# MoonLab-YH/AOD_MEH_HUA

Hardware: AMD Instinct MI355X
Metric: images/sec train+HUA-score, RetinaNet-R50 VOC 512^2 (higher is better)
Workload: dtype bf16x3

## Files before the change

### aod_meh_hua_amd/_C.py

```python
import ctypes as C
import os

import torch

_HERE = os.path.dirname(os.path.abspath(__file__))
LIB_PATH = os.environ.get('AOD_HIP_LIB') or os.path.join(_HERE, 'lib', 'libaodhip.so')


class AodHipError(RuntimeError):
    pass


if not os.path.exists(LIB_PATH):
    raise ImportError(f'{LIB_PATH} is missing: run `python -m aod_meh_hua_amd.build` (hipcc, gfx950). '
                      'There is no CPU fallback for the MEH/HUA hot path.')
lib = C.CDLL(LIB_PATH)


class ConvSeg(C.Structure):
    _fields_ = [('B', C.c_int32), ('H', C.c_int32), ('W', C.c_int32), ('OH', C.c_int32), ('OW', C.c_int32),
                ('src_row0', C.c_int64), ('dst_row0', C.c_int64)]


class ConvDesc(C.Structure):
# ... 42 lines not shown
    'aod_conv2d_plan': (C.c_int, [C.POINTER(ConvDesc), I32, C.c_uint, C.POINTER(ConvPlan)]),
    'aod_conv2d_grouped': (C.c_int, [C.POINTER(ConvDesc), I32, P, P, P, P, P, P, P]),
    'aod_conv2d_ws_map': (C.c_int, [C.POINTER(ConvDesc), P, P, P, P, P, P, P, P, P, P, P, SZ, P, P, P]),
    'aod_conv2d_grouped_map': (C.c_int, [C.POINTER(ConvDesc), I32, P, P, P, P, P, P, P, P, P]),
    'aod_fwd_row_maps': (C.c_int, [C.POINTER(ConvDesc), P, I32, I32, P, P]),
    'aod_conv2d_grouped_fwd_map': (C.c_int, [C.POINTER(ConvDesc), I32, P, P, P, P, P, P]),
    'aod_conv2d_grouped_deal': (C.c_int, [I32, I32, I32, P, P]),
    'aod_conv2d_grouped_map_order': (C.c_int, [C.POINTER(ConvDesc), I32, P, P, P, P, P, P, P, P, P, P]),
    'aod_conv2d_grouped_fwd_map_order': (C.c_int, [C.POINTER(ConvDesc), I32, P, P, P, P, P, P, P]),
    'aod_conv2d_tile_order': (C.c_int, [I32, I32, I32, P, P, P]),
    'aod_halo_conv3x3_applies': (C.c_int, [C.POINTER(ConvDesc)]),
    'aod_halo_conv3x3': (C.c_int, [C.POINTER(ConvDesc), P, P, P, P, P, P, P]),
    'aod_conv2d_wgrad': (C.c_int, [C.POINTER(ConvDesc), P, P, P, P, P]),
    'aod_conv2d_wgrad_splits': (C.c_int, [C.POINTER(ConvDesc)]),
    'aod_conv2d_wgrad_slabs': (C.c_int, [C.POINTER(ConvDesc), P, P, P, I32, I64, P, P]),
    'aod_conv2d_wgrad_slabs_map': (C.c_int, [C.POINTER(ConvDesc), P, P, P, I32, I64, P, P, P]),
    'aod_conv2d_wgrad_group_plan': (C.c_int, [P, I32, P]),
    'aod_conv2d_wgrad_grouped': (C.c_int, [P, I32, P, P, P, P, P, P, P]),
    'aod_conv2d_wgrad_plan': (C.c_int, [P, I32, P, P, P]),
    'aod_conv2d_wgrad_plan_ex': (C.c_int, [P, I32, C.c_uint, C.POINTER(WgradPlan)]),
    'aod_conv2d_wgrad_grouped_map': (C.c_int, [P, I32, P, P, P, P, P, P, P, P]),
    'aod_unpack_wgrad_slabs_grouped': (C.c_int, [I32, P, P, P, P, P, P, P, P, P, P, P, P, P, P, P, P, P]),
    'aod_unpack_wgrad_slabs': (C.c_int, [P, I32, I64, P, I32, I32, I32, I32, I32, I32, P, P, P, P, P, P, P]),
    'aod_conv_row_table_bytes': (SZ, [C.POINTER(ConvDesc)]),
    'aod_conv_row_table': (C.c_int, [C.POINTER(ConvDesc), P, P]),
    'aod_pack_weight_fwd': (C.c_int, [P, P, I32, I32, I32, I32, I32, P]),
    'aod_param_prep': (C.c_int, [P, I32, I32, P]),
    'aod_param_prep_item_bytes': (C.c_int, []),
    'aod_pack_weight_dgrad': (C.c_int, [P, P, I32, I32, I32, I32, I32, P, P]),
    'aod_unpack_wgrad': (C.c_int, [P, P, I32, I32, I32, I32, I32, I32, I32, P, P, P, P, P, P, P]),
    'aod_nchw_f32_to_nhwc_bf16': (C.c_int, [P, P, I32, I32, I32, I32, I32, P]),
    'aod_nchw_f32_to_s2d_bf16': (C.c_int, [P, P, I32, I32, I32, I32, P]),
    'aod_stem_pool_fwd': (C.c_int, [P, P, P, P, P, I32, I32, I32, P]),
    'aod_set_deterministic': (C.c_int, [I32]),
    'aod_get_deterministic': (C.c_int, []),
    'aod_stem_pool_x3_fwd': (C.c_int, [P, P, P, P, P, I32, I32, I32, I32, P]),
    'aod_maxpool3x3s2': (C.c_int, [P, P, I32, I32, I32, I32, P]),
    'aod_upsample2x_add': (C.c_int, [P, P, I32, I32, I32, I32, I32, I32, P]),
    'aod_upsample2x_add_bwd': (C.c_int, [P, P, I32, I32, I32, I32, I32, I32, P]),
    'aod_upsample2x_add_to': (C.c_int, [P, P, P, I32, I32, I32, I32, I32, I32, P]),
    'aod_upsample2x_add_bwd_set': (C.c_int, [P, P, I32, I32, I32, I32, I32, I32, P]),
    'aod_act_bwd': (C.c_int, [P, P, P, P, P, P, P, P, P, P, I64, I32, I32, I32, P]),
    'aod_add_relu': (C.c_int, [P, P, P, I64, P]),
    'aod_pad_cast_colsum': (C.c_int, [P, P, P, P, I64, I32, I32, I32, P]),
    'aod_assign_ws_bytes': (SZ, [I32, I32]),
    'aod_max_iou_assign': (C.c_int, [P, P, I64, I32, P, P, P, I32, F32, F32, F32, I32, I32, P, P, P, P, P, P, P, P, P, I32, P, P]),
# ... 104 lines not shown
```

### aod_meh_hua_amd/csrc/conv.hip

```cpp
#include "common.h"
#include "pointwise.h"
#include "conv_x3p.h"
#include "conv_params.h"

#ifdef AOD_TILE_TIMING
__device__ unsigned long long* g_tile_stamps = nullptr;
extern "C" int aod_dbg_set_tile_stamps(void* buf) { return (int)hipMemcpyToSymbol(HIP_SYMBOL(g_tile_stamps), &buf, sizeof(buf)); }
#define TSTAMP(k) do { if (g_tile_stamps && threadIdx.x == 0) g_tile_stamps[(size_t)blockIdx.x * 16 + (k)] = wall_clock64(); } while (0)
#else
#define TSTAMP(k) do {} while (0)
#endif

__device__ __forceinline__ unsigned udiv_small(unsigned n, unsigned d) {
  unsigned q = (unsigned)((float)n * __builtin_amdgcn_rcpf((float)d));
  const int r = (int)(n - q * d);
  q = r < 0 ? q - 1 : ((unsigned)r >= d ? q + 1 : q);
  return q;
}

__host__ __device__ __forceinline__ void conv_grouped_deal(int bid, int nwg, int ngroups, int mapped, int& tile, int& group) {
  if (!mapped) {
    const int wg = xcd_swizzle(bid, nwg * ngroups);
    tile = wg % nwg; group = wg / nwg;
    return;
// ... 1613 lines not shown
    const float v = dw[si];
    if (clear) dw[si] = 0.f;
    if (w) dot += w[gi] * v;
    g[gi] = accumulate ? g[gi] + v * sc : v * sc;
  }
  if (wdot) {
    dot = wave_sum(dot);
    if ((threadIdx.x & 63) == 0) red[threadIdx.x >> 6] = dot;
    __syncthreads();
    if (threadIdx.x == 0) {
      const float d = red[0] + red[1] + red[2] + red[3];
      wdot[oo] = bn_s1 ? bn_invstd[oo] * (d - bn_mean[oo] * bn_s1[oo]) : d;
    }
  }
}
constexpr int UNP_CH = 1024;
constexpr int UNP_T = 1024;
struct UnpackArgs {
  const float* dw; float* g; const float* scale; const float* w; float* wdot; const float* bn_s1; const float* bn_mean; const float* bn_invstd;
  long long slab_stride;
  int nslabs, O, I, RS, Ipad, accumulate;
  int x3;
};
__device__ __forceinline__ void unpack_row(const UnpackArgs& a, int oo, float* tile, float* red) {
  const float* __restrict__ dw = a.dw;
  float* __restrict__ g = a.g;
  const float* __restrict__ w = a.w;
  const int nslabs = a.nslabs, I = a.I, RS = a.RS, Ipad = a.Ipad, accumulate = a.accumulate;
  const long long slab_stride = a.slab_stride;
  const float sc = a.scale ? a.scale[oo] : 1.f;
  float dot = 0.f;
  const int CH = RS <= 9 ? UNP_CH : (UNP_CH * 9) / RS;
  for (int c0 = 0; c0 < I; c0 += CH) {
    const int nc = min(CH, I - c0);
    for (int i = threadIdx.x; i < nc * RS; i += UNP_T) {
      const int rs = i / nc, c = i - rs * nc;
      float v0 = 0.f, v1 = 0.f, v2 = 0.f, v3 = 0.f;
      {
      const float* src = dw + ((long long)oo * RS + rs) * Ipad + c0 + c;
      int sl = 0;
      for (; sl + 4 <= nslabs; sl += 4) {
        const float a0 = src[(long long)sl * slab_stride], a1 = src[(long long)(sl + 1) * slab_stride];
        const float a2 = src[(long long)(sl + 2) * slab_stride], a3 = src[(long long)(sl + 3) * slab_stride];
        v0 += a0; v1 += a1; v2 += a2; v3 += a3;
      }
      for (; sl < nslabs; ++sl) v0 += src[(long long)sl * slab_stride];
      }
      tile[c * RS + rs] = (v0 + v1) + (v2 + v3);
    }
    __syncthreads();
    const long long g0 = ((long long)oo * I + c0) * RS;
    for (int i = threadIdx.x; i < nc * RS; i += UNP_T) {
      const float v = tile[i];
      if (w) dot += w[g0 + i] * v;
      g[g0 + i] = accumulate ? g[g0 + i] + v * sc : v * sc;
    }
    __syncthreads();
  }
  if (a.wdot) {
    dot = wave_sum(dot);
    if ((threadIdx.x & 63) == 0) red[threadIdx.x >> 6] = dot;
    __syncthreads();
    if (threadIdx.x == 0) {
      float d = 0.f;
      for (int k = 0; k < UNP_T / 64; ++k) d += red[k];
      a.wdot[oo] = a.bn_s1 ? a.bn_invstd[oo] * (d - a.bn_mean[oo] * a.bn_s1[oo]) : d;
    }
  }
}
__global__ __launch_bounds__(UNP_T) void unpack_wgrad_slabs_kernel(const UnpackArgs a) {
  __shared__ float tile[UNP_CH * 9 + 1];
  __shared__ float red[UNP_T / 64];
  unpack_row(a, blockIdx.x, tile, red);
}
struct UnpackGroups { UnpackArgs g[WG_MAXG]; int blk0[WG_MAXG + 1]; };
__global__ __launch_bounds__(UNP_T) void unpack_wgrad_slabs_grouped_kernel(const UnpackGroups gp) {
  __shared__ float tile[UNP_CH * 9 + 1];
  __shared__ float red[UNP_T / 64];
  const int b = blockIdx.x;
  if (b < gp.blk0[1]) unpack_row(gp.g[0], b, tile, red);
  else if (b < gp.blk0[2]) unpack_row(gp.g[1], b - gp.blk0[1], tile, red);
  else if (b < gp.blk0[3]) unpack_row(gp.g[2], b - gp.blk0[2], tile, red);
  else unpack_row(gp.g[3], b - gp.blk0[3], tile, red);
}
struct PrepItem {
  const float* w; const float* gamma; const float* beta; const float* mean; const float* var;
  bf16_t* wf; bf16_t* wd; float* scale; float* shift; float* invstd;
  int O, I, RS, Ipad, Opad, blk0;
  float eps; int flags;
  long long pad2_[2];
};
constexpr int PREP_T = 32, PREP_RS = 9;
__global__ __launch_bounds__(256) void param_prep_kernel(const PrepItem* __restrict__ items, int nitems) {
  __shared__ float tile[PREP_RS][PREP_T][PREP_T + 1];
  int lo = 0, hi = nitems - 1;
  while (lo < hi) {
    const int mid = (lo + hi + 1) >> 1;
    if (items[mid].blk0 <= (int)blockIdx.x) lo = mid; else hi = mid - 1;
  }
  const PrepItem it = items[lo];
  const int lb = blockIdx.x - it.blk0;
  const int t = threadIdx.x;
  if (it.RS > PREP_RS) {
    const long long nf = (long long)it.O * it.RS * it.Ipad, nd = it.wd ? (long long)it.I * it.RS * it.Opad : 0;
    for (int u = 0; u < 8; ++u) {
      const long long i = (long long)lb * 2048 + u * 256 + t;
// ... 155 lines not shown
                                              const float* const* bn_mean, const float* const* bn_invstd, aod_stream_t stream) {
  AOD_CHECK_ARG(n >= 1 && n <= WG_MAXG && dw_slabs && nslabs && slab_stride && g && O && I && R && S && Ipad && accumulate && scale &&
                w_oihw && wdot && bn_s1 && bn_mean && bn_invstd, "unpack_wgrad_slabs_grouped: 1..4 members, no null arrays");
  UnpackGroups gp;
  memset(&gp, 0, sizeof(gp));
  int blk = 0;
  for (int i = 0; i < n; ++i) {
    AOD_CHECK_ARG(dw_slabs[i] && g[i] && nslabs[i] >= 1 && slab_stride[i] > 0 && O[i] >= 1, "unpack_wgrad_slabs_grouped: null / empty member");
    AOD_CHECK_ARG(R[i] * S[i] <= 16, "unpack_wgrad_slabs_grouped: at most 16 taps");
    AOD_CHECK_ARG(!wdot[i] || w_oihw[i], "unpack_wgrad_slabs_grouped: wdot needs the weights");
    AOD_CHECK_ARG(!bn_s1[i] || (wdot[i] && bn_mean[i] && bn_invstd[i]), "unpack_wgrad_slabs_grouped: BN mode needs wdot, mean and invstd");
    UnpackArgs& a = gp.g[i];
    a.dw = dw_slabs[i]; a.g = g[i]; a.scale = scale[i]; a.w = w_oihw[i]; a.wdot = wdot[i]; a.bn_s1 = bn_s1[i]; a.bn_mean = bn_mean[i];
    a.bn_invstd = bn_invstd[i];
    a.slab_stride = slab_stride[i]; a.nslabs = nslabs[i]; a.O = O[i]; a.I = I[i]; a.RS = R[i] * S[i]; a.Ipad = Ipad[i]; a.accumulate = accumulate[i] & 1; a.x3 = (accumulate[i] >> 1) & 1;
    gp.blk0[i] = blk;
    blk += O[i];
  }
  for (int i = n; i <= WG_MAXG; ++i) gp.blk0[i] = i == n ? blk : 0x7fffffff;
  hipLaunchKernelGGL(unpack_wgrad_slabs_grouped_kernel, dim3(blk), dim3(UNP_T), 0, (hipStream_t)stream, gp);
  AOD_LAUNCH_CHECK();
  return 0;
}
extern "C" int aod_unpack_wgrad(float* dw, float* g, int O, int I, int R, int S, int Ipad, int accumulate, int clear_src, const float* scale,
                                const float* w_oihw, float* wdot, const float* bn_s1, const float* bn_mean, const float* bn_invstd,
                                aod_stream_t stream) {
  AOD_CHECK_ARG(dw && g, "unpack_wgrad: null");
  AOD_CHECK_ARG(!wdot || w_oihw, "unpack_wgrad: wdot needs the weights");
  AOD_CHECK_ARG(!bn_s1 || (wdot && bn_mean && bn_invstd), "unpack_wgrad: BN mode needs wdot, mean and invstd");
  if (O == 0) return 0;
  hipLaunchKernelGGL(unpack_wgrad_kernel, dim3(O), dim3(256), 0, (hipStream_t)stream, dw, g, scale, w_oihw, wdot, bn_s1, bn_mean, bn_invstd, O, I,
                     R * S, Ipad, accumulate, clear_src);
  AOD_LAUNCH_CHECK();
  return 0;
}
```

### aod_meh_hua_amd/functional.py

```python
import torch
from torch.autograd import Function

from . import hipops as ho
from .hipops import Seg


def as_rows(x):
    B, C, H, W = x.shape
    xr = x.permute(0, 2, 3, 1)
    if not xr.is_contiguous():
        xr = xr.contiguous()
    return xr.view(B * H * W, C)


def as_nchw(rows, B, H, W):
    return rows.view(B, H, W, rows.shape[1]).permute(0, 3, 1, 2)


def multi_rows(tensors):
    rows = [as_rows(t) for t in tensors]
    if len(rows) == 1:
        t = tensors[0]
        return rows[0], [Seg(t.shape[0], t.shape[2], t.shape[3], 0)]
    rb = rows[0].shape[1] * rows[0].element_size()
# ... 345 lines not shown
MAP_LOG = None
FWD_MAP_LOG = None


def _map_of(dz):
    e = _ROW_MAPS.get(dz.data_ptr())
    return e[0] if e is not None and e[1].shape == dz.shape and e[1].dtype == dz.dtype and ho.sparse_bwd() else None


def _keep_map(dx, rmap):
    if rmap is not None:
        if MAP_LOG is not None:
            MAP_LOG.append((tuple(dx.shape), rmap))
        _WgradQueue.begin_pass()
        _ROW_MAPS[dx.data_ptr()] = (rmap, dx)


class _WgradQueue:
    jobs, seen, task, deferred = [], set(), -1, []
    sparse_jobs = []
    enabled = _os.environ.get('AOD_WGRAD_GROUP', '1') != '0'

    @classmethod
    def flush(cls):
        for name in ('jobs', 'sparse_jobs'):
            jobs = getattr(cls, name)
            setattr(cls, name, [])
            if jobs:
                ho.wgrad_unpack_group(jobs)

    @classmethod
    def _verify(cls):
        deferred, cls.deferred = cls.deferred, []
        for _, pref, t in deferred:
            p = pref()
            if p is None or p.grad is None:
                continue
            g = p.grad
            if g.data_ptr() != t.data_ptr() and g.shape == t.shape:
                g.copy_(t)

    @classmethod
    def _end_of_pass(cls):
        cls.task = -1
        cls.seen.clear()
        _S1_OF.clear()
        _ROW_MAPS.clear()
        cls.flush()
        cls._verify()

    @classmethod
    def begin_pass(cls):
        tid = torch._C._current_graph_task_id()
        if tid != cls.task:
            cls.flush()
            cls.deferred = []
            cls.task = tid
            cls.seen.clear()
            _S1_OF.clear()
            _ROW_MAPS.clear()
            if tid >= 0:
                torch.autograd.Variable._execution_engine.queue_callback(cls._end_of_pass)

    @classmethod
    def submit(cls, job, wid, defer):
        cls.begin_pass()
        if wid in cls.seen or not (defer and cls.enabled) or ho.DETERMINISTIC:
            cls.flush()
            job.run_alone()
            cls.deferred = [e for e in cls.deferred if e[0] != wid]
            cls.seen.add(wid)
            return False
        cls.seen.add(wid)
        name = 'sparse_jobs' if job.zmap is not None else 'jobs'
        q = getattr(cls, name)
        if q and ho.wgrad_group_splits(q + [job]) is None:
            setattr(cls, name, [])
            ho.wgrad_unpack_group(q)
            q = getattr(cls, name)
        q.append(job)
        if len(q) == 4:
            setattr(cls, name, [])
            ho.wgrad_unpack_group(q)
        return True


def _wgrad(x_rows, x_segs, dz, dsegs, R, S, stride, pad, dil, alg, w, O, I, dst, scale=None, bn=None, gamma=None, zmap=None):
    dev = dz.device
    gw = dst if dst is not None else torch.empty(O, I, R, S, dtype=torch.float32, device=dev)
    wdot = torch.empty(O, dtype=torch.float32, device=dev) if bn is not None else None
    job = ho.WgradJob(x_rows, x_segs, dz, dsegs, R, S, stride, pad, dil, alg, O, I, gw.detach(), scale=scale,
                      w=w.detach() if bn is not None else None, wdot=wdot.detach() if wdot is not None else None,
                      bn=tuple(t.detach() for t in bn) if bn is not None else None, zmap=zmap)
    hooked = lambda p: p is not None and bool(p._backward_hooks or getattr(p, '_post_accumulate_grad_hooks', None))
    defer = (R * S <= 9 and w.grad is None and (gamma is None or gamma.grad is None) and not torch.is_grad_enabled()
             and not torch.is_anomaly_enabled() and not hooked(w) and not hooked(gamma))
    if _WgradQueue.submit(job, id(w), defer):
        _WgradQueue.deferred.append((id(w), _weakref.ref(w), job.gw))
        if job.wdot is not None and gamma is not None:
            _WgradQueue.deferred.append((id(w), _weakref.ref(gamma), job.wdot))
    return gw, wdot


class ConvFn(Function):

    @staticmethod
# ... 893 lines not shown
```

### aod_meh_hua_amd/graphs.py

```python
import torch

from . import functional as AF
from . import hipops as ho
from .datasets import DeviceImageBatch

torch.autograd.graph.set_warn_on_accumulate_grad_stream_mismatch(False)
from .models.dense_heads.L_anchor_head import PackedGT


def _pin_caches():
    from . import scoring
    return (dict(ho._ROW_TABLES), dict(ho._DW), dict(ho._SLABS), list(AF.PREP.items.values()), AF.PREP.table, dict(scoring._META))


def _low_memory(dev, frac=0.25):
    try:
        free, total = torch.cuda.mem_get_info(dev)
        return free < frac * total
    except Exception:
        return False


def _unwrap(model):
    return model.module if hasattr(model, 'module') else model


def _plain(data, dev):
    from .mmcv_lite import DataContainer

    def un(x):
        if isinstance(x, DataContainer):
            d = x.data
            return d[0] if isinstance(d, list) and len(d) == 1 else d
        return x
    return {k: un(v) for k, v in data.items()}
# ... 448 lines not shown
```

### aod_meh_hua_amd/hipops.py

```python
import ctypes as C
import os
from dataclasses import dataclass
from typing import List, Optional, Sequence

import torch

from . import _C
from ._C import ConvDesc, ConvSeg, call, lib, ptr, stream


X3 = False
DETERMINISTIC = False


def set_deterministic(on=True):
    global DETERMINISTIC
    rc = lib.aod_set_deterministic(1 if on else 0)
    if rc < 0:
        raise RuntimeError(lib.aod_last_error().decode())
    DETERMINISTIC = bool(on)


def xw(c):
    return 2 * ((c + 31) // 32 * 32)
# ... 295 lines not shown
    if len(_ROW_TABLES) > 512:
        _ROW_TABLES.clear()
    key = (tuple(x_segs), tuple(dz_segs), Cin, Npad, R, S, stride, pad, dil, device.index)
    tab = _ROW_TABLES.get(key)
    if tab is None:
        tab = torch.empty(max(int(_C.lib.aod_conv_row_table_bytes(C.byref(d))), 16), dtype=torch.uint8, device=device)
        call('aod_conv_row_table', C.byref(d), ptr(tab), stream())
        _ROW_TABLES[key] = tab
    return tab


class WgradJob:
    __slots__ = ('x_rows', 'x_segs', 'dz', 'dz_segs', 'R', 'S', 'stride', 'pad', 'dil', 'alg', 'O', 'I', 'gw', 'scale', 'w', 'wdot', 'bn',
                 'desc', 'scope', 'zmap')

    def __init__(self, x_rows, x_segs, dz, dz_segs, R, S, stride, pad, dil, alg, O, I, gw, scale=None, w=None, wdot=None, bn=None, zmap=None):
        self.zmap = zmap
        self.x_rows, self.x_segs, self.dz, self.dz_segs = x_rows, x_segs, dz, dz_segs
        self.R, self.S, self.stride, self.pad, self.dil, self.alg, self.O, self.I = R, S, stride, pad, dil, alg, O, I
        self.gw, self.scale, self.w, self.wdot, self.bn = gw, scale, w, wdot, bn
        self.desc = make_desc(x_rows.shape[1], dz.shape[1], R, S, stride, pad, dil, x_segs, dz_segs, False, False, False)
        self.scope = SCOPE

    def run_alone(self):
        with scope(self.scope):
            self._run_alone()

    def _run_alone(self):
        dw = conv2d_wgrad_rows(self.x_rows, self.x_segs, self.dz, self.dz_segs, self.R, self.S, self.stride, self.pad, self.dil, alg=self.alg,
                               zmap=self.zmap)
        unpack_wgrad(dw, self.O, self.I, grad_oihw=self.gw, scale=self.scale, w_oihw=self.w, want_wdot=self.wdot is not None, bn=self.bn,
                     wdot=self.wdot)


def wgrad_group_splits(jobs):
    n = len(jobs)
    if n > 4 or not SLAB_WGRAD or any(j.R * j.S > 9 for j in jobs):
        return None
    splits = (C.c_int32 * n)()
    rc = _C.lib.aod_conv2d_wgrad_group_plan((C.c_void_p * n)(*[C.addressof(j.desc) for j in jobs]), n, splits)
    return list(splits) if rc == 0 else None


def wgrad_unpack_group(jobs):
    splits = wgrad_group_splits(jobs) if len(jobs) > 1 else None
    if splits is None:
        for j in jobs:
            j.run_alone()
        return
    n = len(jobs)
    dev = jobs[0].dz.device
    lg = 2 if X3 else 1
    strides = [(j.dz.shape[1] // lg) * j.R * j.S * (j.x_rows.shape[1] // lg) for j in jobs]
    offs, tot = [], 0
    for sp, st in zip(splits, strides):
        offs.append(tot)
        tot += sp * st
    buf = _slab_scratch(tot, dev)
    slabs = [buf[o:o + sp * st] for o, sp, st in zip(offs, splits, strides)]
    tabs = [_row_table(j.desc, j.x_segs, j.dz_segs, j.x_rows.shape[1], j.dz.shape[1], j.R, j.S, j.stride, j.pad, j.dil, dev) for j in jobs]
    PA, I32A, I64A = C.c_void_p * n, C.c_int32 * n, C.c_int64 * n
    pv = lambda ts: PA(*[(ptr(t).value if t is not None else None) for t in ts])

    def launch():
        if any(j.zmap is not None for j in jobs):
            call('aod_conv2d_wgrad_grouped_map', PA(*[C.addressof(j.desc) for j in jobs]), n, pv([j.x_rows for j in jobs]),
                 pv([j.dz for j in jobs]), pv(slabs), I32A(*splits), I64A(*strides), pv(tabs), pv([j.zmap for j in jobs]), stream())
            return
        call('aod_conv2d_wgrad_grouped', PA(*[C.addressof(j.desc) for j in jobs]), n, pv([j.x_rows for j in jobs]), pv([j.dz for j in jobs]),
             pv(slabs), I32A(*splits), I64A(*strides), pv(tabs), stream())
    ms = [sum(sg.B * sg.H * sg.W for sg in j.dz_segs) for j in jobs]
    global SCOPE
    SCOPE, prev_scope = jobs[0].scope, SCOPE
    flops = sum(2.0 * m * j.R * j.S * (j.alg[0] * j.alg[1] if j.alg is not None else j.dz.shape[1] * j.x_rows.shape[1]) for m, j in zip(ms, jobs))
    prof_flops('wgrad', (ms[0], sum(j.dz.shape[1] for j in jobs), sum(j.R * j.S * j.x_rows.shape[1] for j in jobs), 10 + n, 1), flops, launch)
    ws = [j.w.contiguous() if (j.wdot is not None and j.w is not None) else None for j in jobs]
    call('aod_unpack_wgrad_slabs_grouped', n, pv(slabs), I32A(*splits), I64A(*strides), pv([j.gw for j in jobs]), I32A(*[j.O for j in jobs]),
         I32A(*[j.I for j in jobs]), I32A(*[j.R for j in jobs]), I32A(*[j.S for j in jobs]), I32A(*[j.x_rows.shape[1] // lg for j in jobs]),
         I32A(*[0] * n), pv([j.scale for j in jobs]), pv(ws), pv([j.wdot for j in jobs]), pv([j.bn[0] if j.bn else None for j in jobs]),
         pv([j.bn[1] if j.bn else None for j in jobs]), pv([j.bn[2] if j.bn else None for j in jobs]), stream())
    SCOPE = prev_scope


def conv2d_wgrad_rows(x_rows, x_segs, dz_rows, dz_segs, R, S, stride=1, pad=0, dil=1, dw=None, alg=None, zmap=None):
    Cin, Npad = x_rows.shape[1], dz_rows.shape[1]
    d = make_desc(Cin, Npad, R, S, stride, pad, dil, x_segs, dz_segs, False, False, False)
    nslabs = 0
    if dw is None and R * S <= (16 if X3 else 9) and SLAB_WGRAD:
        nslabs = int(lib.aod_conv2d_wgrad_splits(C.byref(d)))
    assert not X3 or nslabs, 'x3 weight gradients exist in the slab form only (at most 16 taps)'
    if dw is None and nslabs == 0:
        dw = _dw_scratch(Npad * R * S * Cin, x_rows.device).view(Npad, R, S, Cin)
    tab = _row_table(d, x_segs, dz_segs, Cin, Npad, R, S, stride, pad, dil, x_rows.device)
    if nslabs:
        lg = 2 if X3 else 1
        stride_ = (Npad // lg) * R * S * (Cin // lg)
        slabs = _slab_scratch(nslabs * stride_, x_rows.device).view(nslabs, Npad // lg, R, S, Cin // lg)
        if zmap is not None:
            assert zmap.dtype == torch.uint8 and zmap.numel() == (dz_rows.shape[0] + 63) // 64
            _prof('wgrad', d, lambda: call('aod_conv2d_wgrad_slabs_map', C.byref(d), ptr(x_rows), ptr(dz_rows), ptr(slabs), nslabs, stride_, ptr(tab),
                                           ptr(zmap), stream()), alg)
            return slabs
        _prof('wgrad', d, lambda: call('aod_conv2d_wgrad_slabs', C.byref(d), ptr(x_rows), ptr(dz_rows), ptr(slabs), nslabs, stride_, ptr(tab), stream()), alg)
        return slabs
    _prof('wgrad', d, lambda: call('aod_conv2d_wgrad', C.byref(d), ptr(x_rows), ptr(dz_rows), ptr(dw), ptr(tab), stream()), alg)
    return dw


_DW = {}
_SLABS = {}
SLAB_WGRAD = os.environ.get('AOD_WGRAD_SLABS', '1') != '0'


def _slab_scratch(n, device):
    cap = torch.cuda.is_current_stream_capturing()
    key = (device, torch.cuda.current_stream(device).cuda_stream, _capture_tag() if cap else None)
    buf = _SLABS.pop(key, None)
    if buf is None or buf.numel() < n:
        buf = torch.empty(max(n, (1 << 23) + (1 << 21)), dtype=torch.float32, device=device)
    _SLABS[key] = buf
    while len(_SLABS) > 12:
        _SLABS.pop(next(iter(_SLABS)))
    return buf[:n]


_CAPTURE_SEQ = [0]


def _capture_tag():
    return _CAPTURE_SEQ[0]


def _dw_scratch(n, device):
    buf = _DW.get(device)
    if buf is None or buf.numel() < n:
        buf = torch.zeros(max(n, 1 << 22), dtype=torch.float32, device=device)
        _DW[device] = buf
    return buf[:n]


_ZEROS = {}


def zeros_f32(n, device):
    n_al = (n + 63) // 64 * 64
    ar = _ZEROS.get(device)
    if ar is None or ar[1] + n_al > ar[0].numel():
        ar = [torch.zeros(max(1 << 16, n_al), dtype=torch.float32, device=device), 0]
        _ZEROS[device] = ar
    out = ar[0][ar[1]:ar[1] + n]
    ar[1] += n_al
    return out


def reset_zero_arena():
    _ZEROS.clear()
    _CAPTURE_SEQ[0] += 1


def unpack_wgrad(dw_orsi, O, I, grad_oihw=None, accumulate=False, clear=None, scale=None, w_oihw=None, want_wdot=False, bn=None, wdot=None):
    if dw_orsi.dim() == 5:
        nslabs, Opad, R, S, Ipad = dw_orsi.shape
        if grad_oihw is None:
            grad_oihw = torch.empty(O, I, R, S, dtype=torch.float32, device=dw_orsi.device)
        if wdot is None:
            wdot = torch.empty(O, dtype=torch.float32, device=dw_orsi.device) if want_wdot else None
        call('aod_unpack_wgrad_slabs', ptr(dw_orsi), nslabs, Opad * R * S * Ipad, ptr(grad_oihw), O, I, R, S, Ipad, int(bool(accumulate)), ptr(scale),
             ptr(w_oihw.contiguous()) if want_wdot else None, ptr(wdot), ptr(bn[0]) if bn else None, ptr(bn[1]) if bn else None,
             ptr(bn[2]) if bn else None, stream())
        return (grad_oihw, wdot) if want_wdot else grad_oihw
    Opad, R, S, Ipad = dw_orsi.shape
    if grad_oihw is None:
        grad_oihw = torch.empty(O, I, R, S, dtype=torch.float32, device=dw_orsi.device)
    if clear is None:
        buf = _DW.get(dw_orsi.device)
        clear = buf is not None and dw_orsi.data_ptr() == buf.data_ptr()
    if clear and (O != Opad or I != Ipad):
        pass
    if wdot is None:
        wdot = torch.empty(O, dtype=torch.float32, device=dw_orsi.device) if want_wdot else None
# ... 432 lines not shown
```

### aod_meh_hua_amd/optim.py

```python
import ctypes as C

import torch

from ._C import call, stream


class FusedSGD(torch.optim.Optimizer):

    def __init__(self, params, lr=1e-3, momentum=0.0, dampening=0, weight_decay=0.0, nesterov=False, grad_clip=None, skip_nonfinite=False):
        assert dampening == 0 and not nesterov, 'the AL configs use plain momentum SGD'
        if grad_clip is not None:
            grad_clip = dict(grad_clip)
            if 'max_norm' not in grad_clip:
                raise ValueError(f'grad_clip needs max_norm: {grad_clip}')
            if float(grad_clip.get('norm_type', 2)) != 2.0:
                raise ValueError(f'grad_clip norm_type={grad_clip["norm_type"]!r}: only the 2-norm is implemented')
            if not float(grad_clip['max_norm']) > 0:
                raise ValueError(f'grad_clip max_norm must be positive: {grad_clip["max_norm"]!r}')
        super().__init__(params, dict(lr=lr, momentum=momentum, weight_decay=weight_decay))
        self.grad_scale = 1.0
        self._lr_dev = {}
        self.grad_clip, self.skip_nonfinite = grad_clip, bool(skip_nonfinite)
        self._clip_state, self._clip_ws, self._clip_keep = None, None, []

# ... 10 lines not shown

    def clip_state(self):
        return self._clip_state if self.grad_clip is not None else None

    def device_lr(self):
        for gi, group in enumerate(self.param_groups):
            ent = self._lr_dev.get(gi)
            if ent is None:
                dev = group['params'][0].device
                self._lr_dev[gi] = [torch.full((1,), float(group['lr']), dtype=torch.float32, device=dev), float(group['lr'])]
            elif ent[1] != float(group['lr']):
                ent[0].fill_(float(group['lr']))
                ent[1] = float(group['lr'])
        if self.grad_clip is not None:
            params = [p for g in self.param_groups for p in g['params']]
            if params:
                self._clip_buffers(len(params), params[0].device)

    @torch.no_grad()
    def step(self, closure=None):
        if self._lr_dev and not torch.cuda.is_current_stream_capturing():
            self.device_lr()
        from . import functional as _AF
        _AF._WgradQueue.flush()
        touched, keep = [], []
        batches = []
        for gi, group in enumerate(self.param_groups):
            ps, gs, ms, ns, first = [], [], [], [], None
            for p in group['params']:
                if p.grad is None:
                    continue
                assert p.dtype == torch.float32 and p.is_contiguous()
                g = p.grad if p.grad.is_contiguous() else p.grad.contiguous()
                keep.append(g)
                st = self.state[p]
                is_first = 'momentum_buffer' not in st
                if is_first:
                    st['momentum_buffer'] = torch.empty_like(p)
                if first is None:
                    first = is_first
                if is_first != first:
                    batches.append((gi, group, first, ps, gs, ms, ns))
                    ps, gs, ms, ns, first = [], [], [], [], is_first
                ps.append(p.data_ptr()), gs.append(g.data_ptr()), ms.append(st['momentum_buffer'].data_ptr()), ns.append(p.numel())
                touched.append(p)
            batches.append((gi, group, first, ps, gs, ms, ns))
        coef = None
# ... 42 lines not shown
```

### include/aod_hip.h

```cpp
#ifndef AOD_HIP_H
#define AOD_HIP_H
#include <stddef.h>
#include <stdint.h>

#ifdef __cplusplus
extern "C" {
#endif

typedef void* aod_stream_t;

const char* aod_last_error(void);
int aod_version(void);

typedef struct {
  int32_t B, H, W;
  int32_t OH, OW;
  int64_t src_row0;
  int64_t dst_row0;
} aod_conv_seg_t;

typedef struct {
  int32_t C, N;
  int32_t R, S;
  int32_t stride, pad, dil;
// ... 105 lines not shown
int aod_conv2d_wgrad_plan_ex(const aod_conv_desc_t* const* descs, int n, unsigned flags, aod_wgrad_plan_t* out);
int aod_conv2d_wgrad_plan(const aod_conv_desc_t* const* descs, int n, int32_t* form, int32_t* splits, int32_t* rows_per_split);
int aod_conv2d_wgrad_slabs_map(const aod_conv_desc_t* desc, const void* x, const void* dz, float* slabs, int nslabs, int64_t slab_stride,
                               const void* row_table, const void* dz_map, aod_stream_t stream);
size_t aod_conv_row_table_bytes(const aod_conv_desc_t* desc);
int aod_conv_row_table(const aod_conv_desc_t* desc, void* table, aod_stream_t stream);

int aod_pack_weight_fwd(const float* w_oihw, void* w_packed, int O, int I, int R, int S, int Ipad, aod_stream_t stream);
int aod_pack_weight_dgrad(const float* w_oihw, void* w_packed, int O, int I, int R, int S, int Opad, const float* scale,
                          aod_stream_t stream);
int aod_unpack_wgrad(float* dw_orsi, float* grad_oihw, int O, int I, int R, int S, int Ipad, int accumulate, int clear_src,
                     const float* scale, const float* w_oihw, float* wdot, const float* bn_s1, const float* bn_mean,
                     const float* bn_invstd, aod_stream_t stream);

int aod_unpack_wgrad_slabs(const float* dw_slabs, int nslabs, int64_t slab_stride, float* grad_oihw, int O, int I, int R, int S, int Ipad,
                           int accumulate, const float* scale, const float* w_oihw, float* wdot, const float* bn_s1,
                           const float* bn_mean, const float* bn_invstd, aod_stream_t stream);

int aod_unpack_wgrad_slabs_grouped(int n, const float* const* dw_slabs, const int32_t* nslabs, const int64_t* slab_stride, float* const* g,
                                   const int32_t* O, const int32_t* I, const int32_t* R, const int32_t* S, const int32_t* Ipad,
                                   const int32_t* accumulate, const float* const* scale, const float* const* w_oihw, float* const* wdot,
                                   const float* const* bn_s1, const float* const* bn_mean, const float* const* bn_invstd,
                                   aod_stream_t stream);
int aod_param_prep(const void* items_dev, int nitems, int total_blocks, aod_stream_t stream);
int aod_param_prep_item_bytes(void);

int aod_nchw_f32_to_nhwc_bf16(const float* src, void* dst, int B, int C, int H, int W, int Cpad, aod_stream_t stream);
int aod_nchw_f32_to_s2d_bf16(const float* src, void* dst, int B, int C, int H, int W, aod_stream_t stream);
int aod_stem_pool_fwd(const void* x_s2d, const void* w_packed, const float* scale, const float* shift, void* y, int B, int H2, int W2,
                      aod_stream_t stream);
int aod_maxpool3x3s2(const void* src, void* dst, int B, int H, int W, int C, aod_stream_t stream);
int aod_upsample2x_add(const void* src, void* dst, int B, int h, int w, int C, int H, int W, aod_stream_t stream);
int aod_upsample2x_add_bwd(const void* g_dst, void* g_src_accum, int B, int h, int w, int C, int H, int W, aod_stream_t stream);
int aod_upsample2x_add_to(const void* top, const void* lateral, void* out, int B, int h, int w, int C, int H, int W, aod_stream_t stream);
int aod_upsample2x_add_bwd_set(const void* g_dst, void* g_src, int B, int h, int w, int C, int H, int W, aod_stream_t stream);
int aod_act_bwd(const void* g, const void* a, const void* z, const float* scale, const float* mean, const float* invstd,
                void* dz, void* gmask_out, float* dbeta, float* dgamma, int64_t M, int N, int relu, int g_is_f32,
                aod_stream_t stream);
int aod_pad_cast_colsum(const void* g, const float* relu_out_f32, void* dz, float* colsum, int64_t M, int N, int Npad,
                        int g_is_f32, aod_stream_t stream);
int aod_add_relu(const void* a, const void* b, void* out, int64_t n, aod_stream_t stream);

int aod_halo_conv3x3_applies(const aod_conv_desc_t* desc);
int aod_halo_conv3x3(const aod_conv_desc_t* desc, const void* src, const void* w_packed, void* dst, const float* pre_shift,
                     const void* mask, float* colsum, aod_stream_t stream);

// ... 228 lines not shown
```

Before: 744.3.

## Defer wgrad slab unpacks into one multi-item kernel launched at pass end

Weight-gradient slab reductions are no longer unpacked per job or per group of four. Slabs now live in a per-stream arena and each job records an unpack descriptor; one table-driven kernel unpacks all pending jobs when the backward pass or optimizer step flushes. The kernel finds its item by binary search over block offsets and uses global address-space pointers. This cuts many small kernel launches, but arena slabs stay alive longer, raising memory use, and the table upload has to be handled specially during graph capture.

```diff
diff --git a/aod_meh_hua_amd/_C.py b/aod_meh_hua_amd/_C.py
--- a/aod_meh_hua_amd/_C.py
+++ b/aod_meh_hua_amd/_C.py
@@ -88,6 +88,9 @@
     'aod_conv2d_wgrad_grouped_map': (C.c_int, [P, I32, P, P, P, P, P, P, P, P]),
     'aod_unpack_wgrad_slabs_grouped': (C.c_int, [I32, P, P, P, P, P, P, P, P, P, P, P, P, P, P, P, P, P]),
     'aod_unpack_wgrad_slabs': (C.c_int, [P, I32, I64, P, I32, I32, I32, I32, I32, I32, P, P, P, P, P, P, P]),
+    'aod_unpack_wgrad_multi': (C.c_int, [P, I32, I32, P]),
+    'aod_unpack_wgrad_multi_item_bytes': (C.c_int, []),
+    'aod_unpack_wgrad_multi_item': (C.c_int, [P, I32, I32]),
     'aod_conv_row_table_bytes': (SZ, [C.POINTER(ConvDesc)]),
     'aod_conv_row_table': (C.c_int, [C.POINTER(ConvDesc), P, P]),
     'aod_pack_weight_fwd': (C.c_int, [P, P, I32, I32, I32, I32, I32, P]),
diff --git a/aod_meh_hua_amd/csrc/conv.hip b/aod_meh_hua_amd/csrc/conv.hip
--- a/aod_meh_hua_amd/csrc/conv.hip
+++ b/aod_meh_hua_amd/csrc/conv.hip
@@ -1659,13 +1659,19 @@
   int nslabs, O, I, RS, Ipad, accumulate;
   int x3;
 };
+template <bool GLOBAL> struct UnpFloat { typedef float T; };
+template <> struct UnpFloat<true> { typedef __attribute__((address_space(1))) float T; };
+template <bool TABLE>
 __device__ __forceinline__ void unpack_row(const UnpackArgs& a, int oo, float* tile, float* red) {
-  const float* __restrict__ dw = a.dw;
-  float* __restrict__ g = a.g;
-  const float* __restrict__ w = a.w;
+  typedef typename UnpFloat<TABLE>::T F;
+  const F* __restrict__ dw = (const F*)a.dw;
+  F* __restrict__ g = (F*)a.g;
+  const F* __restrict__ w = (const F*)a.w;
+  const F* const a_scale = (const F*)a.scale; F* const a_wdot = (F*)a.wdot;
+  const F* const a_s1 = (const F*)a.bn_s1; const F* const a_mean = (const F*)a.bn_mean; const F* const a_invstd = (const F*)a.bn_invstd;
   const int nslabs = a.nslabs, I = a.I, RS = a.RS, Ipad = a.Ipad, accumulate = a.accumulate;
   const long long slab_stride = a.slab_stride;
-  const float sc = a.scale ? a.scale[oo] : 1.f;
+  const float sc = a_scale ? a_scale[oo] : 1.f;
   float dot = 0.f;
   const int CH = RS <= 9 ? UNP_CH : (UNP_CH * 9) / RS;
   for (int c0 = 0; c0 < I; c0 += CH) {
@@ -1674,7 +1680,7 @@
       const int rs = i / nc, c = i - rs * nc;
       float v0 = 0.f, v1 = 0.f, v2 = 0.f, v3 = 0.f;
       {
-      const float* src = dw + ((long long)oo * RS + rs) * Ipad + c0 + c;
+      const F* src = dw + ((long long)oo * RS + rs) * Ipad + c0 + c;
       int sl = 0;
       for (; sl + 4 <= nslabs; sl += 4) {
         const float a0 = src[(long long)sl * slab_stride], a1 = src[(long long)(sl + 1) * slab_stride];
@@ -1694,31 +1700,50 @@
     }
     __syncthreads();
   }
-  if (a.wdot) {
+  if (a_wdot) {
     dot = wave_sum(dot);
     if ((threadIdx.x & 63) == 0) red[threadIdx.x >> 6] = dot;
     __syncthreads();
     if (threadIdx.x == 0) {
       float d = 0.f;
       for (int k = 0; k < UNP_T / 64; ++k) d += red[k];
-      a.wdot[oo] = a.bn_s1 ? a.bn_invstd[oo] * (d - a.bn_mean[oo] * a.bn_s1[oo]) : d;
+      a_wdot[oo] = a_s1 ? a_invstd[oo] * (d - a_mean[oo] * a_s1[oo]) : d;
     }
   }
 }
 __global__ __launch_bounds__(UNP_T) void unpack_wgrad_slabs_kernel(const UnpackArgs a) {
   __shared__ float tile[UNP_CH * 9 + 1];
   __shared__ float red[UNP_T / 64];
-  unpack_row(a, blockIdx.x, tile, red);
+  unpack_row<false>(a, blockIdx.x, tile, red);
 }
 struct UnpackGroups { UnpackArgs g[WG_MAXG]; int blk0[WG_MAXG + 1]; };
 __global__ __launch_bounds__(UNP_T) void unpack_wgrad_slabs_grouped_kernel(const UnpackGroups gp) {
   __shared__ float tile[UNP_CH * 9 + 1];
   __shared__ float red[UNP_T / 64];
   const int b = blockIdx.x;
-  if (b < gp.blk0[1]) unpack_row(gp.g[0], b, tile, red);
-  else if (b < gp.blk0[2]) unpack_row(gp.g[1], b - gp.blk0[1], tile, red);
-  else if (b < gp.blk0[3]) unpack_row(gp.g[2], b - gp.blk0[2], tile, red);
-  else unpack_row(gp.g[3], b - gp.blk0[3], tile, red);
+  if (b < gp.blk0[1]) unpack_row<false>(gp.g[0], b, tile, red);
+  else if (b < gp.blk0[2]) unpack_row<false>(gp.g[1], b - gp.blk0[1], tile, red);
+  else if (b < gp.blk0[3]) unpack_row<false>(gp.g[2], b - gp.blk0[2], tile, red);
+  else unpack_row<false>(gp.g[3], b - gp.blk0[3], tile, red);
+}
+struct UnpackItem { UnpackArgs a; int blk0; int pad_; };
+static_assert(sizeof(UnpackItem) == 112 && offsetof(UnpackItem, blk0) == 104, "UnpackItem layout is mirrored by hipops._UnpackRec");
+__host__ __device__ __forceinline__ int unpack_multi_item(const int* first, int stride_ints, int nitems, int block) {
+  int lo = 0, hi = nitems - 1;
+  while (lo < hi) {
+    const int mid = (lo + hi + 1) >> 1;
+    if (first[(long long)mid * stride_ints] <= block) lo = mid; else hi = mid - 1;
+  }
+  return lo;
+}
+__global__ __launch_bounds__(UNP_T) void unpack_wgrad_multi_kernel(const UnpackItem* __restrict__ items, int nitems) {
+  __shared__ float tile[UNP_CH * 9 + 1];
+  __shared__ float red[UNP_T / 64];
+  const int i = unpack_multi_item(&items[0].blk0, (int)(sizeof(UnpackItem) / sizeof(int)), nitems, (int)blockIdx.x);
+  const UnpackItem it = items[i];
+  const int oo = (int)blockIdx.x - it.blk0;
+  if (oo >= it.a.O) return;
+  unpack_row<true>(it.a, oo, tile, red);
 }
 struct PrepItem {
   const float* w; const float* gamma; const float* beta; const float* mean; const float* var;
@@ -1920,6 +1945,19 @@
   AOD_LAUNCH_CHECK();
   return 0;
 }
+extern "C" int aod_unpack_wgrad_multi(const void* items_dev, int nitems, int nblocks, aod_stream_t stream) {
+  AOD_CHECK_ARG(items_dev && nitems >= 0 && nblocks >= 0, "unpack_wgrad_multi: bad args");
+  AOD_CHECK_ARG((nitems == 0) == (nblocks == 0) && nblocks >= nitems, "unpack_wgrad_multi: every item owns at least one block");
+  if (nitems == 0) return 0;
+  hipLaunchKernelGGL(unpack_wgrad_multi_kernel, dim3(nblocks), dim3(UNP_T), 0, (hipStream_t)stream, (const UnpackItem*)items_dev, nitems);
+  AOD_LAUNCH_CHECK();
+  return 0;
+}
+extern "C" int aod_unpack_wgrad_multi_item_bytes(void) { return (int)sizeof(UnpackItem); }
+extern "C" int aod_unpack_wgrad_multi_item(const int32_t* first_block, int nitems, int block) {
+  AOD_CHECK_ARG(first_block && nitems >= 1 && block >= 0 && first_block[0] == 0, "unpack_wgrad_multi_item: bad args");
+  return unpack_multi_item(first_block, 1, nitems, block);
+}
 extern "C" int aod_unpack_wgrad(float* dw, float* g, int O, int I, int R, int S, int Ipad, int accumulate, int clear_src, const float* scale,
                                 const float* w_oihw, float* wdot, const float* bn_s1, const float* bn_mean, const float* bn_invstd,
                                 aod_stream_t stream) {
diff --git a/aod_meh_hua_amd/functional.py b/aod_meh_hua_amd/functional.py
--- a/aod_meh_hua_amd/functional.py
+++ b/aod_meh_hua_amd/functional.py
@@ -391,12 +391,21 @@
     enabled = _os.environ.get('AOD_WGRAD_GROUP', '1') != '0'
 
     @classmethod
+    def _launch(cls, jobs):
+        ho.wgrad_unpack_group(jobs, defer_unpack=ho.UNPACK_MULTI)
+
+    @classmethod
     def flush(cls):
         for name in ('jobs', 'sparse_jobs'):
             jobs = getattr(cls, name)
             setattr(cls, name, [])
             if jobs:
-                ho.wgrad_unpack_group(jobs)
+                cls._launch(jobs)
+
+    @classmethod
+    def finish(cls):
+        cls.flush()
+        ho.unpack_multi_flush()
 
     @classmethod
     def _verify(cls):
@@ -415,14 +424,14 @@
         cls.seen.clear()
         _S1_OF.clear()
         _ROW_MAPS.clear()
-        cls.flush()
+        cls.finish()
         cls._verify()
 
     @classmethod
     def begin_pass(cls):
         tid = torch._C._current_graph_task_id()
         if tid != cls.task:
-            cls.flush()
+            cls.finish()
             cls.deferred = []
             cls.task = tid
             cls.seen.clear()
@@ -435,7 +444,13 @@
     def submit(cls, job, wid, defer):
         cls.begin_pass()
         if wid in cls.seen or not (defer and cls.enabled) or ho.DETERMINISTIC:
-            cls.flush()
+            late = ho.UNPACK_MULTI and defer and cls.enabled and wid not in cls.seen
+            if late:
+                cls.flush()
+                job.run_alone(defer_unpack=True)
+                cls.seen.add(wid)
+                return True
+            cls.finish()
             job.run_alone()
             cls.deferred = [e for e in cls.deferred if e[0] != wid]
             cls.seen.add(wid)
@@ -445,12 +460,12 @@
         q = getattr(cls, name)
         if q and ho.wgrad_group_splits(q + [job]) is None:
             setattr(cls, name, [])
-            ho.wgrad_unpack_group(q)
+            cls._launch(q)
             q = getattr(cls, name)
         q.append(job)
         if len(q) == 4:
             setattr(cls, name, [])
-            ho.wgrad_unpack_group(q)
+            cls._launch(q)
         return True
 
 
diff --git a/aod_meh_hua_amd/graphs.py b/aod_meh_hua_amd/graphs.py
--- a/aod_meh_hua_amd/graphs.py
+++ b/aod_meh_hua_amd/graphs.py
@@ -10,7 +10,8 @@
 
 def _pin_caches():
     from . import scoring
-    return (dict(ho._ROW_TABLES), dict(ho._DW), dict(ho._SLABS), list(AF.PREP.items.values()), AF.PREP.table, dict(scoring._META))
+    return (dict(ho._ROW_TABLES), dict(ho._DW), dict(ho._SLABS), list(AF.PREP.items.values()), AF.PREP.table, dict(scoring._META),
+            ho.take_capture_arenas())
 
 
 def _low_memory(dev, frac=0.25):
diff --git a/aod_meh_hua_amd/hipops.py b/aod_meh_hua_amd/hipops.py
--- a/aod_meh_hua_amd/hipops.py
+++ b/aod_meh_hua_amd/hipops.py
@@ -341,13 +341,17 @@
         self.desc = make_desc(x_rows.shape[1], dz.shape[1], R, S, stride, pad, dil, x_segs, dz_segs, False, False, False)
         self.scope = SCOPE
 
-    def run_alone(self):
+    def run_alone(self, defer_unpack=False):
         with scope(self.scope):
-            self._run_alone()
-
-    def _run_alone(self):
+            self._run_alone(defer_unpack)
+
+    def _run_alone(self, defer_unpack=False):
         dw = conv2d_wgrad_rows(self.x_rows, self.x_segs, self.dz, self.dz_segs, self.R, self.S, self.stride, self.pad, self.dil, alg=self.alg,
-                               zmap=self.zmap)
+                               zmap=self.zmap, pass_long=defer_unpack)
+        if defer_unpack and dw.dim() == 5:
+            nslabs, Opad, R, S, Ipad = dw.shape
+            _defer_unpack(dw, nslabs, Opad * R * S * Ipad, self, Ipad)
+            return
         unpack_wgrad(dw, self.O, self.I, grad_oihw=self.gw, scale=self.scale, w_oihw=self.w, want_wdot=self.wdot is not None, bn=self.bn,
                      wdot=self.wdot)
 
@@ -361,11 +365,11 @@
     return list(splits) if rc == 0 else None
 
 
-def wgrad_unpack_group(jobs):
+def wgrad_unpack_group(jobs, defer_unpack=False):
     splits = wgrad_group_splits(jobs) if len(jobs) > 1 else None
     if splits is None:
         for j in jobs:
-            j.run_alone()
+            j.run_alone(defer_unpack)
         return
     n = len(jobs)
     dev = jobs[0].dz.device
@@ -375,7 +379,7 @@
     for sp, st in zip(splits, strides):
         offs.append(tot)
         tot += sp * st
-    buf = _slab_scratch(tot, dev)
+    buf = _arena(dev).alloc(tot, dev) if defer_unpack else _slab_scratch(tot, dev)
     slabs = [buf[o:o + sp * st] for o, sp, st in zip(offs, splits, strides)]
     tabs = [_row_table(j.desc, j.x_segs, j.dz_segs, j.x_rows.shape[1], j.dz.shape[1], j.R, j.S, j.stride, j.pad, j.dil, dev) for j in jobs]
     PA, I32A, I64A = C.c_void_p * n, C.c_int32 * n, C.c_int64 * n
@@ -393,6 +397,11 @@
     SCOPE, prev_scope = jobs[0].scope, SCOPE
     flops = sum(2.0 * m * j.R * j.S * (j.alg[0] * j.alg[1] if j.alg is not None else j.dz.shape[1] * j.x_rows.shape[1]) for m, j in zip(ms, jobs))
     prof_flops('wgrad', (ms[0], sum(j.dz.shape[1] for j in jobs), sum(j.R * j.S * j.x_rows.shape[1] for j in jobs), 10 + n, 1), flops, launch)
+    if defer_unpack:
+        for j, sl, sp, st in zip(jobs, slabs, splits, strides):
+            _defer_unpack(sl, sp, st, j, j.x_rows.shape[1] // lg)
+        SCOPE = prev_scope
+        return
     ws = [j.w.contiguous() if (j.wdot is not None and j.w is not None) else None for j in jobs]
     call('aod_unpack_wgrad_slabs_grouped', n, pv(slabs), I32A(*splits), I64A(*strides), pv([j.gw for j in jobs]), I32A(*[j.O for j in jobs]),
          I32A(*[j.I for j in jobs]), I32A(*[j.R for j in jobs]), I32A(*[j.S for j in jobs]), I32A(*[j.x_rows.shape[1] // lg for j in jobs]),
@@ -401,7 +410,7 @@
     SCOPE = prev_scope
 
 
-def conv2d_wgrad_rows(x_rows, x_segs, dz_rows, dz_segs, R, S, stride=1, pad=0, dil=1, dw=None, alg=None, zmap=None):
+def conv2d_wgrad_rows(x_rows, x_segs, dz_rows, dz_segs, R, S, stride=1, pad=0, dil=1, dw=None, alg=None, zmap=None, pass_long=False):
     Cin, Npad = x_rows.shape[1], dz_rows.shape[1]
     d = make_desc(Cin, Npad, R, S, stride, pad, dil, x_segs, dz_segs, False, False, False)
     nslabs = 0
@@ -414,7 +423,8 @@
     if nslabs:
         lg = 2 if X3 else 1
         stride_ = (Npad // lg) * R * S * (Cin // lg)
-        slabs = _slab_scratch(nslabs * stride_, x_rows.device).view(nslabs, Npad // lg, R, S, Cin // lg)
+        slabs = (_arena(x_rows.device).alloc(nslabs * stride_, x_rows.device) if pass_long else _slab_scratch(nslabs * stride_, x_rows.device))
+        slabs = slabs.view(nslabs, Npad // lg, R, S, Cin // lg)
         if zmap is not None:
             assert zmap.dtype == torch.uint8 and zmap.numel() == (dz_rows.shape[0] + 63) // 64
             _prof('wgrad', d, lambda: call('aod_conv2d_wgrad_slabs_map', C.byref(d), ptr(x_rows), ptr(dz_rows), ptr(slabs), nslabs, stride_, ptr(tab),
@@ -443,6 +453,145 @@
     return buf[:n]
 
 
+UNPACK_MULTI = os.environ.get('AOD_UNPACK_MULTI', '1') != '0'
+ARENA_CHUNK = 1 << 25
+ARENA_STATS = dict(peak_bytes=0, launches=0, items=0, blocks=0, slab_bytes=0, log=[])
+
+
+class _UnpackRec(C.Structure):
+    _fields_ = [('dw', C.c_void_p), ('g', C.c_void_p), ('scale', C.c_void_p), ('w', C.c_void_p), ('wdot', C.c_void_p), ('bn_s1', C.c_void_p),
+                ('bn_mean', C.c_void_p), ('bn_invstd', C.c_void_p), ('slab_stride', C.c_int64), ('nslabs', C.c_int32), ('O', C.c_int32),
+                ('I', C.c_int32), ('RS', C.c_int32), ('Ipad', C.c_int32), ('accumulate', C.c_int32), ('x3', C.c_int32), ('pad_', C.c_int32),
+                ('blk0', C.c_int32), ('pad2_', C.c_int32)]
+
+
+class _SlabArena:
+    __slots__ = ('chunks', 'cur', 'off', 'used', 'recs', 'keep', 'blocks', 'tables')
+
+    def __init__(self):
+        self.chunks, self.cur, self.off, self.used, self.recs, self.keep, self.blocks, self.tables = [], 0, 0, 0, [], [], 0, []
+
+    def alloc(self, n, device):
+        n_al = (n + 63) // 64 * 64
+        while self.cur < len(self.chunks) and self.off + n_al > self.chunks[self.cur].numel():
+            self.cur, self.off = self.cur + 1, 0
+        if self.cur == len(self.chunks):
+            self.chunks.append(torch.empty(max(n_al, ARENA_CHUNK), dtype=torch.float32, device=device))
+        out = self.chunks[self.cur][self.off:self.off + n]
+        self.off += n_al
+        self.used += n_al
+        return out
+
+    def reset(self):
+        ARENA_STATS['peak_bytes'] = max(ARENA_STATS['peak_bytes'], 4 * self.used)
+        self.cur = self.off = self.used = self.blocks = 0
+        self.recs, self.keep = [], []
+
+
+_ARENAS = {}
+_UNPACK_TABLES = {}
+_TABLE_UPLOADS = []
+
+
+def set_unpack_multi(on=True):
+    global UNPACK_MULTI
+    unpack_multi_flush()
+    UNPACK_MULTI = bool(on)
+
+
+def _arena(device):
+    cap = torch.cuda.is_current_stream_capturing()
+    key = (device, torch.cuda.current_stream(device).cuda_stream, _capture_tag() if cap else None)
+    ar = _ARENAS.pop(key, None)
+    if ar is None:
+        ar = _SlabArena()
+    _ARENAS[key] = ar
+    if len(_ARENAS) > 4:
+        for k in [k for k, a in _ARENAS.items() if not a.recs and a is not ar][:len(_ARENAS) - 4]:
+            del _ARENAS[k]
+    return ar
+
+
+def _defer_unpack(slabs, nslabs, slab_stride, job, Ipad):
+    assert job.R * job.S <= 16 and nslabs >= 1 and slab_stride > 0 and job.O >= 1
+    assert job.wdot is None or job.w is not None, 'wdot needs the weights'
+    assert not job.bn or job.wdot is not None, 'BN mode needs wdot'
+    ar = _arena(slabs.device)
+    w = job.w.contiguous() if (job.wdot is not None and job.w is not None) else None
+    r = _UnpackRec()
+    r.dw, r.g = slabs.data_ptr(), job.gw.data_ptr()
+    r.scale, r.w, r.wdot = (None if t is None else t.data_ptr() for t in (job.scale, w, job.wdot))
+    r.bn_s1, r.bn_mean, r.bn_invstd = (t.data_ptr() for t in job.bn) if job.bn else (None, None, None)
+    r.slab_stride, r.nslabs, r.O, r.I, r.RS, r.Ipad, r.accumulate, r.x3 = slab_stride, nslabs, job.O, job.I, job.R * job.S, Ipad, 0, 0
+    r.blk0 = ar.blocks
+    ar.blocks += job.O
+    ar.recs.append(r)
+    ar.keep.append((job.gw, job.scale, w, job.wdot, job.bn))
+
+
+def _launch_unpack_multi(ar, device):
+    recs = (_UnpackRec * len(ar.recs))(*ar.recs)
+    raw = bytes(recs)
+    assert len(raw) == len(ar.recs) * int(lib.aod_unpack_wgrad_multi_item_bytes()), 'UnpackItem layout'
+    if torch.cuda.is_current_stream_capturing():
+        pool, n_al = _TABLE_POOL[0], (len(raw) + 255) // 256 * 256
+        if pool is None or pool.device != device or _TABLE_POOL[1] + n_al > pool.numel():
+            for r in ar.recs:
+                call('aod_unpack_wgrad_slabs', r.dw, r.nslabs, r.slab_stride, r.g, r.O, r.I, r.RS, 1, r.Ipad, r.accumulate, r.scale, r.w, r.wdot,
+                     r.bn_s1, r.bn_mean, r.bn_invstd, stream())
+            return
+        table = pool[_TABLE_POOL[1]:_TABLE_POOL[1] + len(raw)]
+        _TABLE_POOL[1] += n_al
+        _TABLE_UPLOADS.append((table, raw))
+        ar.tables.append(table)
+    else:
+        table = _UNPACK_TABLES.pop(raw, None)
+        if table is None:
+            table = torch.frombuffer(bytearray(raw), dtype=torch.uint8).to(device)
+        _UNPACK_TABLES[raw] = table
+        while len(_UNPACK_TABLES) > 8:
+            _UNPACK_TABLES.pop(next(iter(_UNPACK_TABLES)))
+    ARENA_STATS.update(launches=ARENA_STATS['launches'] + 1, items=len(ar.recs), blocks=ar.blocks,
+                       slab_bytes=sum(4 * r.nslabs * r.O * r.RS * r.I for r in ar.recs))
+    ARENA_STATS['log'] = ARENA_STATS['log'][-7:] + [(ARENA_STATS['items'], ARENA_STATS['blocks'], ARENA_STATS['slab_bytes'], 4 * ar.used)]
+    call('aod_unpack_wgrad_multi', ptr(table), len(ar.recs), ar.blocks, stream())
+
+
+def unpack_multi_flush():
+    for key, ar in list(_ARENAS.items()):
+        if not ar.recs:
+            continue
+        dev, st = key[0], key[1]
+        try:
+            if torch.cuda.current_stream(dev).cuda_stream == st:
+                _launch_unpack_multi(ar, dev)
+            else:
+                with torch.cuda.stream(torch.cuda.ExternalStream(st, device=dev)):
+                    _launch_unpack_multi(ar, dev)
+        finally:
+            ar.reset()
+
+
+def take_capture_arenas():
+    out = [_ARENAS.pop(k) for k in [k for k, a in _ARENAS.items() if k[2] is not None and not a.recs]]
+    return [(a.chunks, a.tables) for a in out]
+
+
+_TABLE_POOL = [None, 0]
+TABLE_POOL_BYTES = 1 << 18
+
+
+def _upload_tables():
+    if not torch.cuda.is_available() or not torch.cuda.is_initialized() or torch.cuda.is_current_stream_capturing():
+        return
+    ups = list(_TABLE_UPLOADS)
+    del _TABLE_UPLOADS[:]
+    for table, raw in ups:
+        table.copy_(torch.frombuffer(bytearray(raw), dtype=torch.uint8))
+    if _TABLE_POOL[0] is None or _TABLE_POOL[1] or _TABLE_POOL[0].device.index != torch.cuda.current_device():
+        _TABLE_POOL[0], _TABLE_POOL[1] = torch.empty(TABLE_POOL_BYTES, dtype=torch.uint8, device=torch.device('cuda', torch.cuda.current_device())), 0
+
+
 _CAPTURE_SEQ = [0]
 
 
@@ -475,6 +624,7 @@
 def reset_zero_arena():
     _ZEROS.clear()
     _CAPTURE_SEQ[0] += 1
+    _upload_tables()
 
 
 def unpack_wgrad(dw_orsi, O, I, grad_oihw=None, accumulate=False, clear=None, scale=None, w_oihw=None, want_wdot=False, bn=None, wdot=None):
diff --git a/aod_meh_hua_amd/optim.py b/aod_meh_hua_amd/optim.py
--- a/aod_meh_hua_amd/optim.py
+++ b/aod_meh_hua_amd/optim.py
@@ -56,7 +56,7 @@
         if self._lr_dev and not torch.cuda.is_current_stream_capturing():
             self.device_lr()
         from . import functional as _AF
-        _AF._WgradQueue.flush()
+        _AF._WgradQueue.finish()
         touched, keep = [], []
         batches = []
         for gi, group in enumerate(self.param_groups):
diff --git a/include/aod_hip.h b/include/aod_hip.h
--- a/include/aod_hip.h
+++ b/include/aod_hip.h
@@ -151,6 +151,9 @@
                                    const int32_t* accumulate, const float* const* scale, const float* const* w_oihw, float* const* wdot,
                                    const float* const* bn_s1, const float* const* bn_mean, const float* const* bn_invstd,
                                    aod_stream_t stream);
+int aod_unpack_wgrad_multi(const void* items_dev, int nitems, int nblocks, aod_stream_t stream);
+int aod_unpack_wgrad_multi_item_bytes(void);
+int aod_unpack_wgrad_multi_item(const int32_t* first_block, int nitems, int block);
 int aod_param_prep(const void* items_dev, int nitems, int total_blocks, aod_stream_t stream);
 int aod_param_prep_item_bytes(void);
 
```

Result: no change. 747.4 (median of 6 runs) (+0.4%).
